# Victarry/Image-Generation-models

Measured on AMD Instinct MI355X. Metric: ddpm_cifar10_32x32_train_images_per_sec, higher is better.
Workload: dtype bf16; 1 GPU; DDPM CIFAR-10 32x32, UNet 128/1-2-4, T=1000 (BASELINE configs[1]): train step B=128/GPU + hipGraph denoise step B=64; per_gpu_batch=128, global_batch=128, parallelism=dp1, step_launch=hipGraph replay, denoise_batch=64, rccl_ranks=1, state_finite=True, matmul=bf16 MFMA, fp32 accumulate

## Files before the change

### image-generation-models_amd/csrc/conv_pw.hip

```cpp
#include "tr_common.h"

#ifndef MI_PW_PABL
#define MI_PW_PABL 0
#endif
#ifndef MI_PW_GNSABL
#define MI_PW_GNSABL 0
#endif
#ifndef MI_PW_FXABL
#define MI_PW_FXABL 0
#endif
#ifdef MI_PW_TIMING
__device__ uint32_t g_pw_ts[1024 * 4 * 5 * 64];
__device__ __forceinline__ uint32_t pw_wlane(uint32_t val, uint32_t lane, uint32_t v) {
    uint32_t keep;
    asm volatile("s_mov_b32 %1, m0\n\ts_mov_b32 m0, %3\n\ts_nop 0\n\tv_writelane_b32 %0, %2, m0\n\ts_mov_b32 m0, %1"
                 : "+v"(v), "=&s"(keep) : "s"(__builtin_amdgcn_readfirstlane(val)), "s"(__builtin_amdgcn_readfirstlane(lane)));
    return v;
}
extern "C" int mi_debug_pw_ts(uint32_t* host_out) { return (int)hipMemcpyFromSymbol(host_out, HIP_SYMBOL(g_pw_ts), sizeof(g_pw_ts)); }
#endif

namespace {

typedef uint32_t u32x2 __attribute__((ext_vector_type(2)));
// ... 1436 lines not shown
    auto unit = [&](int jt, auto chc, auto setc) {
        constexpr int ch = decltype(chc)::value, set = decltype(setc)::value;
        const bool last_unit = ch == NCH - 1 && jt + 1 >= jt1;
        if (!last_unit) {
            if constexpr (ch + 1 < NCH) load_wu(jt, ch + 1, std::integral_constant<int, set ^ 1>{});
            else load_wu(jt + 1, 0, std::integral_constant<int, set ^ 1>{});
        }
        bf16x8 XC[2][NBLK];
#pragma unroll
        for (int i = 0; i < NBLK; ++i) XC[0][i] = lds_b128p(xa[i] + ch * XB);
        static_for<0, 8>([&](auto uc) {
            constexpr int u = decltype(uc)::value;
            if constexpr (u + 1 < 8) {
                constexpr int un = u + 1;
#pragma unroll
                for (int i = 0; i < NBLK; ++i) XC[un & 1][i] = lds_b128p((xa[i] ^ ((un & 3) * 32)) + (un >> 2) * XH + ch * XB);
            }
#pragma unroll
            for (int i = 0; i < NBLK; ++i)
                acc[i] = __builtin_amdgcn_mfma_f32_32x32x16_bf16(__builtin_bit_cast(bf16x8, WB[set][u]), XC[u & 1][i], acc[i], 0, 0, 0);
            __builtin_amdgcn_sched_barrier(0);
        });
        if constexpr (ch == NCH - 1) {
            const int n0 = jt * 128;
            if (n0 + 32 * wv < a.Nc) {
#pragma unroll
                for (int rq = 0; rq < 4; ++rq) {
                    const int ck = 8 * wv + 2 * rq + (l >> 5);
                    f32x4 bq = {0.f, 0.f, 0.f, 0.f};
                    if (a.bias) bq = *reinterpret_cast<const f32x4*>(a.bias + n0 + 4 * ck);
#pragma unroll
                    for (int i = 0; i < NBLK; ++i) {
                        const int p = i * 32 + (l & 31);
                        *(lds_u32x2n*)(uintptr_t)(lds0 + STG + p * 256 + ((ck ^ ((p & 15) << 1)) << 3)) =
                            u32x2{pack_bf16(acc[i][4 * rq] + bq.x, acc[i][4 * rq + 1] + bq.y), pack_bf16(acc[i][4 * rq + 2] + bq.z, acc[i][4 * rq + 3] + bq.w)};
                    }
                }
            }
#pragma unroll
            for (int i = 0; i < NBLK; ++i)
#pragma unroll
                for (int r = 0; r < 16; ++r) acc[i][r] = 0.f;
        }
        asm volatile("s_waitcnt vmcnt(0)" ::: "memory");
        static_for<0, 8>([&](auto uc) { landed16(WB[set ^ 1][decltype(uc)::value]); });
        if constexpr (ch == NCH - 1) {
            const int n0 = jt * 128;
            __syncthreads();
            {
                const int j = t & 15, col = n0 + 8 * j;
                if (col < a.Nc) {
#pragma unroll
                    for (int it = 0; it < PXT / 16; ++it) {
                        const int p = it * 16 + (t >> 4);
                        const u32x4 o = *(lds_u32x4n*)(uintptr_t)(lds0 + STG + p * 256 + (((2 * j) ^ ((p & 15) << 1)) << 3));
                        *reinterpret_cast<u32x4*>(a.y + ((size_t)m0 + p) * a.ldy + col) = o;
                    }
                }
            }
            __syncthreads();
        }
    };
    auto cotile = [&](int jt, auto jpc) {
        constexpr int JP = decltype(jpc)::value;
        static_for<0, NCH>([&](auto chc) {
            constexpr int ch = decltype(chc)::value;
            unit(jt, chc, std::integral_constant<int, (JP * NCH + ch) & 1>{});
        });
    };
    for (int jt = jt0; jt < jt1; jt += 2) {
        cotile(jt, std::integral_constant<int, 0>{});
        if (jt + 1 < jt1) cotile(jt + 1, std::integral_constant<int, 1>{});
    }
}

struct GtClass { unsigned long long dyq, dxq, wtq; int ntap, ao, bo, pad_; };
struct GtArgs {
    const uint16_t* x; const uint16_t* w; const float* bias; const float* res; void* y; uint16_t* y16; int ldy16;
    int M, K, Nc, ldx, ldy, ldr, accumulate, gx, gy;
    int IH, IW, lgGW, lgGHW, si, so, OH, OW;
    GtClass cls[4];
};

template <bool OUT16, int PXT, bool F32 = false>
__global__ __launch_bounds__(256, 2) void conv_gt_kernel(const GtArgs a) {
    MI_PRIO_UP();
    static_assert(!F32 || !OUT16, "exact-fp32 mode writes fp32");
    constexpr int ESZ = F32 ? 4 : 2, EPP = 16 / ESZ, HCH = 8 * EPP;
    extern __shared__ __attribute__((aligned(16))) uint8_t lds_raw[];
    const uint32_t lds0 = (uint32_t)(uintptr_t)lds_raw;
    constexpr int NBLK = PXT / 32;
    constexpr int XH = PXT * 128;
    constexpr int XB = 2 * XH;
    const int t = threadIdx.x, l = t & 63;
    const int wv = __builtin_amdgcn_readfirstlane(t >> 6);
    int bx = blockIdx.x, by = blockIdx.y;
    if (a.gy > 1 && a.gx % 8 == 0) {
        const int id = blockIdx.x, xcd = id & 7, slot = id >> 3;
        bx = xcd * (a.gx >> 3) + slot / a.gy; by = slot % a.gy;
    }
    const GtClass cl = a.cls[blockIdx.z];
    const int m0 = bx * PXT, n0 = by * 128;
    const int NB = a.Nc >> 5, KQ = a.K / (2 * EPP), kc64 = a.K / HCH;
    const int nhc = cl.ntap * kc64, nchunks = (nhc + 1) >> 1;
    const bool live = n0 + 32 * wv < a.Nc;
    const int nb = min((n0 >> 5) + wv, NB - 1);

    int pbase[NBLK], iy0[NBLK], ix0[NBLK];
#pragma unroll
    for (int j = 0; j < NBLK; ++j) {
        const int m = m0 + 8 * (wv + 4 * j) + (l >> 3);
        const int n = m >> a.lgGHW, r = m & ((1 << a.lgGHW) - 1);
        pbase[j] = n * a.IH * a.IW; iy0[j] = (r >> a.lgGW) * a.si; ix0[j] = (r & ((1 << a.lgGW) - 1)) * a.si;
    }
    const uint8_t* zero = reinterpret_cast<const uint8_t*>(g_zero_page3) + (l & 7) * 16;
    auto stage_x = [&](int ch) {
#pragma unroll
        for (int h = 0; h < 2; ++h) {
            const int hc = min(2 * ch + h, 2 * nchunks - 1);
            const bool pad_half = hc >= nhc;
            const int hcc = min(hc, nhc - 1), tp = hcc / kc64, c0 = (hcc - tp * kc64) * HCH;
            const int dy = (int)((cl.dyq >> (4 * tp)) & 15) - 8, dx = (int)((cl.dxq >> (4 * tp)) & 15) - 8;
#pragma unroll
            for (int j = 0; j < NBLK; ++j) {
                const int px = 8 * (wv + 4 * j) + (l >> 3);
                const int iy = iy0[j] + dy, ix = ix0[j] + dx;
                const bool ok = !pad_half && (unsigned)iy < (unsigned)a.IH && (unsigned)ix < (unsigned)a.IW;
                size_t off = (size_t)(pbase[j] + iy * a.IW + ix) * a.ldx + c0 + ((l & 7) ^ ((px >> 1) & 7)) * EPP;
                asm volatile("" : "+v"(off));
                const uint8_t* src = ok ? reinterpret_cast<const uint8_t*>(a.x) + off * ESZ : zero;
                glds16(src, lds0 + (ch & 1) * XB + h * XH + (wv + 4 * j) * 1024);
            }
        }
    };
    const uint8_t* wbase = reinterpret_cast<const uint8_t*>(a.w) + (size_t)nb * KQ * 1024;
    const uint32_t tap_bytes = (uint32_t)NB * KQ * 1024;
    const uint32_t wl16 = l * 16;
    u32x4 WB[2][8];
    auto load_w = [&](int ch, auto setc) {
        constexpr int set = decltype(setc)::value;
        static_for<0, 2>([&](auto hcst) {
            constexpr int h = decltype(hcst)::value;
            const int hcc = min(2 * min(ch, nchunks - 1) + h, nhc - 1), tp = hcc / kc64, c0 = (hcc - tp * kc64) * HCH;
            const int wt = (int)((cl.wtq >> (4 * tp)) & 15);
            const uint64_t q = (uint64_t)(uintptr_t)(wbase + (size_t)wt * tap_bytes + (size_t)(c0 / (2 * EPP)) * 1024);
            const uint32_t lo = __builtin_amdgcn_readfirstlane((uint32_t)q), hi = __builtin_amdgcn_readfirstlane((uint32_t)(q >> 32));
            const uint64_t sb = ((uint64_t)hi << 32) | lo;
            static_for<0, 4>([&](auto uc) { gload16s<decltype(uc)::value * 1024>(WB[set][4 * h + decltype(uc)::value], sb, wl16); });
        });
    };
    uint32_t xa[NBLK];
#pragma unroll
    for (int i = 0; i < NBLK; ++i) {
        const int px = i * 32 + (l & 31);
        xa[i] = lds0 + px * 128 + (((l >> 5) * 16) ^ (((px >> 1) & 7) * 16));
    }
    f32x16 acc[NBLK];
#pragma unroll
    for (int i = 0; i < NBLK; ++i)
#pragma unroll
        for (int r = 0; r < 16; ++r) acc[i][r] = 0.f;

    stage_x(0);
    load_w(0, std::integral_constant<int, 0>{});
    asm volatile("s_waitcnt vmcnt(0)" ::: "memory");
    static_for<0, 8>([&](auto uc) { landed16(WB[0][decltype(uc)::value]); });
    auto chunk = [&](int ch, auto setc) {
        constexpr int set = decltype(setc)::value;
        asm volatile("s_waitcnt lgkmcnt(0)" ::: "memory");
        __builtin_amdgcn_s_barrier();
        asm volatile("" ::: "memory");
        if (ch + 1 < nchunks) {
            stage_x(ch + 1);
            load_w(ch + 1, std::integral_constant<int, set ^ 1>{});
        }
        const uint32_t xb = (ch & 1) * XB;
        bf16x8 XC[2][NBLK];
#pragma unroll
        for (int i = 0; i < NBLK; ++i) XC[0][i] = lds_b128p(xa[i] + xb);
        static_for<0, 8>([&](auto uc) {
            constexpr int u = decltype(uc)::value;
            if constexpr (u + 1 < 8) {
                constexpr int un = u + 1;
#pragma unroll
                for (int i = 0; i < NBLK; ++i) XC[un & 1][i] = lds_b128p((xa[i] ^ ((un & 3) * 32)) + (un >> 2) * XH + xb);
            }
#pragma unroll
            for (int i = 0; i < NBLK; ++i) {
                if constexpr (F32) {
                    const f32x4 wv4 = __builtin_bit_cast(f32x4, WB[set][u]), xv4 = __builtin_bit_cast(f32x4, XC[u & 1][i]);
#pragma unroll
                    for (int jj = 0; jj < 4; ++jj) acc[i] = __builtin_amdgcn_mfma_f32_32x32x2f32(wv4[jj], xv4[jj], acc[i], 0, 0, 0);
                } else
                acc[i] = __builtin_amdgcn_mfma_f32_32x32x16_bf16(__builtin_bit_cast(bf16x8, WB[set][u]), XC[u & 1][i], acc[i], 0, 0, 0);
            }
            __builtin_amdgcn_sched_barrier(0);
        });
        asm volatile("s_waitcnt vmcnt(0)" ::: "memory");
        static_for<0, 8>([&](auto uc) { landed16(WB[set ^ 1][decltype(uc)::value]); });
    };
    for (int ch = 0; ch < nchunks; ch += 2) {
        chunk(ch, std::integral_constant<int, 0>{});
        if (ch + 1 < nchunks) chunk(ch + 1, std::integral_constant<int, 1>{});
    }

    __syncthreads();
    typedef __attribute__((address_space(3))) f32x4 lds_f32x4;
    if (live) {
#pragma unroll
        for (int i = 0; i < NBLK; ++i) {
            const int p = i * 32 + (l & 31);
#pragma unroll
            for (int rq = 0; rq < 4; ++rq) {
                const int ck = 8 * wv + 2 * rq + (l >> 5);
                *(lds_f32x4*)(uintptr_t)(lds0 + p * 512 + ((ck ^ (p & 31)) << 4)) =
                    f32x4{acc[i][4 * rq], acc[i][4 * rq + 1], acc[i][4 * rq + 2], acc[i][4 * rq + 3]};
            }
        }
    }
    __syncthreads();
    const int j = t & 15, col = n0 + 8 * j;
    if (col >= a.Nc) return;
    f32x4 b0 = {0.f, 0.f, 0.f, 0.f}, b1 = b0;
    if (a.bias) { b0 = *reinterpret_cast<const f32x4*>(a.bias + col); b1 = *reinterpret_cast<const f32x4*>(a.bias + col + 4); }
#pragma unroll
    for (int it = 0; it < PXT / 16; ++it) {
        const int p = it * 16 + (t >> 4);
        const int mm = m0 + p, n = mm >> a.lgGHW, r = mm & ((1 << a.lgGHW) - 1);
        const size_t m = ((size_t)n * a.OH + (r >> a.lgGW) * a.so + cl.ao) * a.OW + (r & ((1 << a.lgGW) - 1)) * a.so + cl.bo;
        f32x4 v0 = *(lds_f32x4*)(uintptr_t)(lds0 + p * 512 + (((2 * j) ^ (p & 31)) << 4)) + b0;
        f32x4 v1 = *(lds_f32x4*)(uintptr_t)(lds0 + p * 512 + (((2 * j + 1) ^ (p & 31)) << 4)) + b1;
        if (a.res) {
            v0 += *reinterpret_cast<const f32x4*>(a.res + m * a.ldr + col);
            v1 += *reinterpret_cast<const f32x4*>(a.res + m * a.ldr + col + 4);
        }
        if constexpr (OUT16) {
            uint16_t* yp = reinterpret_cast<uint16_t*>(a.y) + m * a.ldy + col;
            if (a.accumulate) {
                const u32x4 o = *reinterpret_cast<const u32x4*>(yp);
                v0 += f32x4{__uint_as_float(o.x << 16), __uint_as_float(o.x & 0xffff0000u), __uint_as_float(o.y << 16), __uint_as_float(o.y & 0xffff0000u)};
                v1 += f32x4{__uint_as_float(o.z << 16), __uint_as_float(o.z & 0xffff0000u), __uint_as_float(o.w << 16), __uint_as_float(o.w & 0xffff0000u)};
            }
            *reinterpret_cast<u32x4*>(yp) = u32x4{pack_bf16(v0.x, v0.y), pack_bf16(v0.z, v0.w), pack_bf16(v1.x, v1.y), pack_bf16(v1.z, v1.w)};
        } else {
            float* yp = reinterpret_cast<float*>(a.y) + m * a.ldy + col;
            if (a.accumulate) { v0 += *reinterpret_cast<const f32x4*>(yp); v1 += *reinterpret_cast<const f32x4*>(yp + 4); }
            *reinterpret_cast<f32x4*>(yp) = v0;
            *reinterpret_cast<f32x4*>(yp + 4) = v1;
            if (a.y16)
                *reinterpret_cast<u32x4*>(a.y16 + m * a.ldy16 + col) =
                    u32x4{pack_bf16(v0.x, v0.y), pack_bf16(v0.z, v0.w), pack_bf16(v1.x, v1.y), pack_bf16(v1.z, v1.w)};
        }
    }
}

bool pw1_ok(const MiConvDesc* d, bool f32 = false, bool in32 = false) {
    if (in32) {
        if (d->KH != 1 || d->KW != 1 || d->pad != 0 || d->stride != 1 || d->mode != 1 || d->IH != d->OH || d->IW != d->OW) return false;
        if (d->K % 128 || d->K1 % 128 || d->K1 <= 0 || d->K1 > d->K || d->Nc % 64 || d->ldx % 4 || (d->K1 != d->K && d->ldx2 % 4)) return false;
        return ((long)d->N * d->OH * d->OW) % 128 == 0;
    }
    if (f32) {
        if (d->KH != 1 || d->KW != 1 || d->pad != 0 || d->stride != 1 || d->mode != 0 || d->IH != d->OH || d->IW != d->OW) return false;
        if (d->K % 64 || d->K1 % 64 || d->K1 <= 0 || d->K1 > d->K || d->Nc % 64 || d->ldx % 4 || (d->K1 != d->K && d->ldx2 % 4)) return false;
        return ((long)d->N * d->OH * d->OW) % 128 == 0;
    }
    if (d->KH != 1 || d->KW != 1 || d->pad != 0 || d->stride != 1 || d->mode != 1) return false;
    if (d->IH != d->OH || d->IW != d->OW) return false;
    if (d->K % 128 || d->K1 % 128 || d->K1 <= 0 || d->K1 > d->K || d->Nc % 64 || d->ldx % 8 || (d->K1 != d->K && d->ldx2 % 8)) return false;
    return ((long)d->N * d->OH * d->OW) % 128 == 0;
}

struct PwGn { const float* sums; const float* gamma; const float* beta; const float* temb; int ldt, G; float eps; };

static int pw_launch(const char* who, const MiConvDesc* d, const void* x, const void* x2, const void* w_frag_bf16, const float* bias,
                     const float* residual, void* y, int out_bf16, int var, float* gsum, const float* coef, void* stream,
                     const PwGn* gn = nullptr, bool in32 = false, bool f32 = false) {
    PwArgs a{};
    if (!d || !x || !w_frag_bf16 || !y) return mi_set_error(-1, "%s: null argument", who);
    const int pt = pw_pick_tile(d, var, &a.TH, &a.TI, in32, f32, &a.ksplit);
    if (!pt) return mi_set_error(-1, "%s: descriptor not supported by the private-weight-stream conv kernel", who);
    int dev_ = 0;
    (void)hipGetDevice(&dev_);
    if (a.ksplit > 1) {
        uint8_t* ws = reinterpret_cast<uint8_t*>(g_pw_sk_ws[dev_ & 63].load(std::memory_order_acquire));
        a.sk_flag = reinterpret_cast<int*>(ws); a.sk_part = reinterpret_cast<float*>(ws + PW_SK_FLAG_BYTES);
#ifdef MI_PW_SK_ABL
        a.sk_flag = nullptr;
#endif
    }
    if (d->K1 != d->K && !x2) return mi_set_error(-1, "%s: two-source split without x2", who);
    if ((((uintptr_t)x | (uintptr_t)(x2 ? x2 : x) | (uintptr_t)w_frag_bf16) & 15) != 0) return mi_set_error(-1, "%s: operands must be 16-byte aligned", who);
    if (d->ldy % 8 || (residual && d->ldr % 4)) return mi_set_error(-1, "%s: output pixel stride must be a multiple of 8, the residual's of 4", who);
    if (var >= 2 && (a.TI != 1 || d->K1 != d->K))
        return mi_set_error(-1, "%s: the fused variants need one image per tile and one source", who);
    if (var == 2 && (!coef || ((uintptr_t)coef & 15)))
        return mi_set_error(-1, "%s: the fused variant needs a 16-byte aligned coefficient tensor", who);
    if (var == 3) {
        if (!gn || !gn->sums || !gn->gamma || !gn->beta || gn->G <= 0 || d->K % gn->G || (d->K / gn->G) % 16 || d->K / gn->G > 64 || d->K / gn->G == 48)
            return mi_set_error(-1, "%s: sums, gamma, beta; K / G in {16, 32, 64}", who);
        if ((((uintptr_t)gn->gamma | (uintptr_t)gn->beta | (uintptr_t)gn->sums) & 7) || ((uintptr_t)gn->sums & 15) || (gn->temb && (((uintptr_t)gn->temb & 15) || gn->ldt % 4)))
            return mi_set_error(-1, "%s: misaligned GroupNorm operands", who);
        a.sums = gn->sums; a.gamma = gn->gamma; a.beta = gn->beta; a.temb = gn->temb; a.ldt = gn->ldt; a.cpg = d->K / gn->G;
        a.cpg_magic = pw_magic(a.cpg); a.ng = gn->G; a.hw = d->OH * d->OW; a.eps = gn->eps; a.icnt = 1.0 / (MI_GSUM_SCALE * (double)a.hw * (double)a.cpg);
    }
    if (var == 1 && (!gsum || d->Nc % 16)) return mi_set_error(-1, "%s: GroupNorm sums need Nc %% 16 == 0 and a sum buffer", who);
    a.x = (const uint16_t*)x; a.x2 = (const uint16_t*)(x2 ? x2 : x); a.w = (const uint16_t*)w_frag_bf16; a.bias = bias; a.res = residual; a.y = y;
    a.N = d->N; a.H = d->OH; a.W = d->OW; a.K = d->K; a.Nc = d->Nc; a.K1 = d->K1; a.ldx = d->ldx; a.ldx2 = x2 ? d->ldx2 : d->ldx;
    a.ldy = d->ldy; a.ldr = d->ldr; a.accumulate = d->accumulate; a.flip = d->transposed ? 1 : 0;
    a.gsum = gsum; a.coef = coef;
// ... 369 lines not shown
    a.ln_out = (uint16_t*)ln_bf16; a.ldl = ldl;
    hipStream_t st = (hipStream_t)stream;
#define MI_LNPW1_GO(PX, NC, G) do { \
        static MiPerDevice once_; \
        once_.run([] { (void)hipFuncSetAttribute((const void*)ln_conv1x1_pw_kernel<PX, NC, G>, hipFuncAttributeMaxDynamicSharedMemorySize, (int)lnpw1_lds(PX, NC)); }); \
        a.gx = a.M / PX; \
        hipLaunchKernelGGL((ln_conv1x1_pw_kernel<PX, NC, G>), dim3((unsigned)(a.gx * (G ? a.gy : 1))), dim3(256), lnpw1_lds(PX, NC), st, a); } while (0)
#define MI_LNPW1_PICK(PX, NC) do { if (a.M / PX < 512) MI_LNPW1_GO(PX, NC, true); else MI_LNPW1_GO(PX, NC, false); } while (0)
    if (d->K == 128) { if (a.M / 128 >= 512) MI_LNPW1_GO(128, 1, false); else MI_LNPW1_PICK(64, 1); }
    else if (d->K == 256) MI_LNPW1_PICK(64, 2);
    else MI_LNPW1_PICK(64, 4);
#undef MI_LNPW1_PICK
#undef MI_LNPW1_GO
    MI_LAUNCH_CHECK();
    return 0;
}

static int ilog2_exact(int v) { int lg = 0; while ((1 << lg) < v) ++lg; return (1 << lg) == v ? lg : -1; }

static bool gt_plan(const MiConvDesc* d, GtArgs& a, int* ncls, int* pxt) {
    if (!d || (d->mode != 1 && d->mode != 0) || d->K1 != d->K || d->K % 64 || d->Nc % 64 || d->ldx % (d->mode == 1 ? 8 : 4)) return false;
    const int k = d->KH, s = d->stride, p = d->pad;
    if (d->KW != k || k * k > 16 || k < 1 || (s != 1 && s != 2) || p < 0 || p > 7) return false;
    if ((long)d->Nc * d->K * (d->mode == 1 ? 2 : 4) * k * k >= (1L << 31)) return false;
    int GH, GW;
    *ncls = 0;
    if (!d->transposed) {
        if (d->OH != (d->IH + 2 * p - k) / s + 1 || d->OW != (d->IW + 2 * p - k) / s + 1) return false;
        GH = d->OH; GW = d->OW; a.si = s; a.so = 1;
        GtClass c{};
        for (int ky = 0; ky < k; ++ky)
            for (int kx = 0; kx < k; ++kx) {
                const int tp = c.ntap++;
                c.dyq |= (unsigned long long)(ky - p + 8) << (4 * tp); c.dxq |= (unsigned long long)(kx - p + 8) << (4 * tp);
                c.wtq |= (unsigned long long)(ky * k + kx) << (4 * tp);
            }
        a.cls[(*ncls)++] = c;
    } else {
        if (d->OH != s * d->IH || d->OW != s * d->IW) return false;
        GH = d->OH / s; GW = d->OW / s; a.si = 1; a.so = s;
        for (int cy = 0; cy < s; ++cy)
            for (int cx = 0; cx < s; ++cx) {
                GtClass c{};
                c.ao = cy; c.bo = cx;
                for (int ky = (cy + p) % s; ky < k; ky += s)
                    for (int kx = (cx + p) % s; kx < k; kx += s) {
                        const int dy = (cy + p - ky) / s, dx = (cx + p - kx) / s;
                        if (dy < -8 || dy > 7 || dx < -8 || dx > 7) return false;
                        const int tp = c.ntap++;
                        c.dyq |= (unsigned long long)(dy + 8) << (4 * tp); c.dxq |= (unsigned long long)(dx + 8) << (4 * tp);
                        c.wtq |= (unsigned long long)(ky * k + kx) << (4 * tp);
                    }
                if (c.ntap == 0) return false;
                a.cls[(*ncls)++] = c;
            }
    }
    a.lgGW = ilog2_exact(GW); a.lgGHW = ilog2_exact(GH * GW);
    if (a.lgGW < 0 || a.lgGHW < 0) return false;
    a.M = d->N * GH * GW; a.K = d->K; a.Nc = d->Nc; a.IH = d->IH; a.IW = d->IW; a.OH = d->OH; a.OW = d->OW;
    if (a.M % 64) return false;
    a.gy = (d->Nc + 127) / 128;
    const bool small = a.M % 128 != 0 || (long)(a.M / 128) * a.gy * *ncls < 256;
    *pxt = small ? 64 : 128;
    a.gx = a.M / *pxt;
    return true;
}
extern "C" int mi_conv_gt_supported(const MiConvDesc* d) {
    GtArgs a{};
    int ncls, pxt;
    return gt_plan(d, a, &ncls, &pxt) ? 1 : 0;
}
static int gt_launch(const MiConvDesc* d, const void* x, const void* w_frag, const float* bias, const float* residual,
                     void* y, int out_bf16, void* y_bf16, int ldy16, void* stream);
extern "C" int mi_conv_gt(const MiConvDesc* d, const void* x, const void* w_frag, const float* bias, const float* residual,
                          void* y, int out_bf16, void* stream) {
    return gt_launch(d, x, w_frag, bias, residual, y, out_bf16, nullptr, 0, stream);
}
extern "C" int mi_conv_gt_dual(const MiConvDesc* d, const void* x, const void* w_frag, const float* bias, const float* residual,
                               float* y, void* y_bf16, int ldy16, void* stream) {
    MI_REQUIRE(y_bf16 && ldy16 % 8 == 0 && (((uintptr_t)y_bf16) & 15) == 0 && d && !d->accumulate && d->mode == 1,
               "bf16 copy: bf16 mode, 16-byte aligned, ldy16 % 8 == 0, no accumulate");
    return gt_launch(d, x, w_frag, bias, residual, y, 0, y_bf16, ldy16, stream);
}
static int gt_launch(const MiConvDesc* d, const void* x, const void* w_frag, const float* bias, const float* residual,
                     void* y, int out_bf16, void* y_bf16, int ldy16, void* stream) {
    MI_REQUIRE(d && x && w_frag && y, "null argument");
    GtArgs a{};
    int ncls, pxt;
    MI_REQUIRE(gt_plan(d, a, &ncls, &pxt), "descriptor not supported by the tap-gather kernel (one source, K and Nc % 64 == 0, "
               "k * k <= 16 taps, stride 1 / 2, power-of-two grids, N*GH*GW % 64 == 0)");
    MI_REQUIRE((((uintptr_t)x | (uintptr_t)w_frag) & 15) == 0, "operands must be 16-byte aligned");
    MI_REQUIRE(d->ldy % 8 == 0 && (!residual || d->ldr % 4 == 0), "pixel strides: y % 8, residual % 4");
    MI_REQUIRE(d->mode == 1 || !out_bf16, "the exact-fp32 kernel writes fp32");
    a.x = (const uint16_t*)x; a.w = (const uint16_t*)w_frag; a.bias = bias; a.res = residual; a.y = y; a.y16 = (uint16_t*)y_bf16; a.ldy16 = ldy16;
    a.ldx = d->ldx; a.ldy = d->ldy; a.ldr = d->ldr; a.accumulate = d->accumulate;
    dim3 grid((unsigned)a.gx, (unsigned)a.gy, (unsigned)ncls);
    if (a.gy > 1 && a.gx % 8 == 0) grid = dim3((unsigned)(a.gx * a.gy), 1, (unsigned)ncls);
    hipStream_t st = (hipStream_t)stream;
#define MI_GT_GO(O16, PX, F) do { \
        static MiPerDevice once_; \
        once_.run([] { (void)hipFuncSetAttribute((const void*)conv_gt_kernel<O16, PX, F>, hipFuncAttributeMaxDynamicSharedMemorySize, 64 * 1024); }); \
        hipLaunchKernelGGL((conv_gt_kernel<O16, PX, F>), grid, dim3(256), (size_t)(PX == 128 ? 64 : 32) * 1024, st, a); } while (0)
    if (d->mode == 0) { if (pxt == 128) MI_GT_GO(false, 128, true); else MI_GT_GO(false, 64, true); }
    else if (pxt == 128) { if (out_bf16) MI_GT_GO(true, 128, false); else MI_GT_GO(false, 128, false); }
    else { if (out_bf16) MI_GT_GO(true, 64, false); else MI_GT_GO(false, 64, false); }
#undef MI_GT_GO
    MI_LAUNCH_CHECK();
    return 0;
}
extern "C" int mi_conv_gt_tile(const MiConvDesc* d, int* pxt, int* ncls) {
    GtArgs a{};
    return gt_plan(d, a, ncls, pxt) ? 0 : -1;
}
```

### image-generation-models_amd/src/ops/lib.py

```python
from __future__ import annotations

import ctypes as C
import os

_PKG_ROOT = os.path.dirname(os.path.dirname(os.path.dirname(os.path.abspath(__file__))))
_LIB = None


def library_path() -> str:
    return os.environ.get("MI_DDPM_LIB", os.path.join(_PKG_ROOT, "lib", "libmi_ddpm.so"))


class MiConvDesc(C.Structure):
    _fields_ = [(n, C.c_int) for n in (
        "N", "IH", "IW", "OH", "OW", "K", "Nc", "KH", "KW", "stride", "pad", "transposed", "w_kn", "mode",
        "K1", "ldx", "ldx2", "ldy", "ldr", "accumulate")]


class MiWgradDesc(C.Structure):
    _fields_ = [(n, C.c_int) for n in (
        "N", "GH", "GW", "DH", "DW", "Ci", "Cj", "KH", "KW", "stride", "pad", "gather_i", "mode", "I1",
        "ldp", "ldp2", "ldq")]


class MiGnDesc(C.Structure):
    _fields_ = [("N", C.c_int), ("HW", C.c_int), ("C", C.c_int), ("G", C.c_int), ("eps", C.c_float),
                ("ldx", C.c_int), ("ldy", C.c_int), ("ldr", C.c_int)]


class MiRowSum(C.Structure):
    _fields_ = [("src", C.c_void_p), ("dst", C.c_void_p), ("rows", C.c_int), ("cols", C.c_int), ("ld", C.c_int), ("pad_", C.c_int)]


WGRAD_STORE = 1


class MiPcnnConvDesc(C.Structure):
    _fields_ = ([(n, C.c_int) for n in ("N", "H", "W", "Cin", "ldx", "Cout", "ldy", "ntaps")]
                + [(n, C.c_int * 25) for n in ("tap_dy", "tap_dx", "tap_w")]
                + [(n, C.c_int) for n in ("w_sk", "w_sc", "C2", "ldx2", "w2_sk", "w2_sc", "epi", "elu_in", "accumulate", "gate_C",
                                          "ldpre", "ldcond", "ldr", "ldaux", "mode")])


ROWSUM_MAX = 16
LATENT_DISC_NMAX = 1024
LATENT_DISC_LN_NMAX = 65536
_P, _I, _F, _Z = C.c_void_p, C.c_int, C.c_float, C.c_size_t

SIGNATURES = {
    "mi_conv_igemm": [C.POINTER(MiConvDesc), _P, _P, _P, _P, _P, _P, _P],
    "mi_conv_igemm_bf16w": [C.POINTER(MiConvDesc), _P, _P, _P, _P, _P, _P, _P],
    "mi_conv_igemm_bf16w_io": [C.POINTER(MiConvDesc), _P, _P, _P, _P, _P, _P, _I, _P],
    "mi_conv_igemm_bf16w_io_supported": [C.POINTER(MiConvDesc)],
    "mi_conv_gt_supported": [C.POINTER(MiConvDesc)],
    "mi_conv_gt_tile": [C.POINTER(MiConvDesc), C.POINTER(C.c_int), C.POINTER(C.c_int)],
    "mi_conv_gt": [C.POINTER(MiConvDesc), _P, _P, _P, _P, _P, _I, _P],
    "mi_conv_gt_dual": [C.POINTER(MiConvDesc), _P, _P, _P, _P, _P, _P, _I, _P],
    "mi_conv_igemm_tile": [C.POINTER(MiConvDesc), C.POINTER(C.c_int), C.POINTER(C.c_int)],
    "mi_conv3x3_bf16w": [C.POINTER(MiConvDesc), _P, _P, _P, _P, _P, _P, _P],
    "mi_conv3x3_bf16w_supported": [C.POINTER(MiConvDesc)],
    "mi_conv3x3_bf16w_uses_splitk": [C.POINTER(MiConvDesc)],
    "mi_conv3x3_bf16w_tile": [C.POINTER(MiConvDesc), _I, C.POINTER(C.c_int), C.POINTER(C.c_int), C.POINTER(C.c_int)],
    "mi_conv3x3_wgrad_tile": [C.POINTER(MiWgradDesc), C.POINTER(C.c_int), C.POINTER(C.c_int)],
    "mi_debug_wgrad3x3_phase": [_I],
    "mi_conv3x3_wgrad_tr_supported": [C.POINTER(MiWgradDesc)],
    "mi_conv3x3_wgrad_tr_splits": [C.POINTER(MiWgradDesc)],
    "mi_conv3x3_wgrad_tr": [C.POINTER(MiWgradDesc), _P, _P, _P, _P, _P, _Z, _P],
    "mi_conv3x3_wgrad_tr_batch": [_I, C.POINTER(MiWgradDesc), C.POINTER(_P), C.POINTER(_P), C.POINTER(_P), C.POINTER(_P), _P, _Z, _P],
    "mi_debug_wgrad_tr_phase": [_I],
    "mi_conv1x1_wgrad_tr_supported": [C.POINTER(MiWgradDesc), _I],
    "mi_conv1x1_wgrad_tr_batch": [_I, C.POINTER(MiWgradDesc), C.POINTER(_I), C.POINTER(_P), C.POINTER(_P), C.POINTER(_P), C.POINTER(_P),
                                  C.POINTER(_P), _P, _Z, _P],
    "mi_debug_wgrad1x1_tr_phase": [_I],
    "mi_conv_s2_wgrad_tr_supported": [C.POINTER(MiWgradDesc)],
    "mi_conv_s2_wgrad_tr_batch": [_I, C.POINTER(MiWgradDesc), C.POINTER(_P), C.POINTER(_P), C.POINTER(_P), _P, _Z, _P],
    "mi_conv_s2_wgrad_f32_supported": [C.POINTER(MiWgradDesc)],
    "mi_conv_s2_wgrad_f32": [C.POINTER(MiWgradDesc), _P, _P, _P, _P, _Z, _P],
    "mi_debug_wgrad_s2_tr_phase": [_I],
    "mi_conv3x3_wgrad_tr_batch_ex": [_I, C.POINTER(MiWgradDesc), C.POINTER(_P), C.POINTER(_P), C.POINTER(_P), C.POINTER(_P), _P, _Z, _P, C.c_uint],
    "mi_conv1x1_wgrad_tr_batch_ex": [_I, C.POINTER(MiWgradDesc), C.POINTER(_I), C.POINTER(_P), C.POINTER(_P), C.POINTER(_P), C.POINTER(_P),
                                     C.POINTER(_P), _P, _Z, _P, C.c_uint],
    "mi_conv_s2_wgrad_tr_batch_ex": [_I, C.POINTER(MiWgradDesc), C.POINTER(_P), C.POINTER(_P), C.POINTER(_P), _P, _Z, _P, C.c_uint],
    "mi_zero_ranges": [_P, _I, _P, _P],
    "mi_debug_spin": [_I, _I, _P, _Z, _I, _P],
    "mi_debug_clock_probe": [_I, _I, _P, _P],
    "mi_pack_weights_tile": [],
    "mi_conv3x3_bf16w_io_gnsums": [C.POINTER(MiConvDesc), _P, _P, _P, _P, _P, _P, _I, _P, _P],
    "mi_gn_coef_from_sums": [_I, _I, _I, _I, _F, _P, _P, _P, _P, _I, _P, _P, _P],
    "mi_gn_mish_apply_sums": [C.POINTER(MiGnDesc), _P, _P, _P, _P, _P, _I, _P, _P, _I, _P, _I, _P, _P],
    "mi_conv3x3_bf16w_io_dual": [C.POINTER(MiConvDesc), _P, _P, _P, _P, _P, _P, _P, _I, _I, _P],
    "mi_conv3x3_gn_mish_sums": [C.POINTER(MiConvDesc), _P, _P, _P, _P, _P, _I, _I, _F, _P, _P, _P, _I, _P],
    "mi_debug_wgrad1x1_tr_blocks": [_I],
    "mi_debug_wgrad_tr_blocks": [_I],
    "mi_conv3x3_bf16w_io": [C.POINTER(MiConvDesc), _P, _P, _P, _P, _P, _P, _I, _P],
    "mi_conv3x3_wgrad_io": [C.POINTER(MiWgradDesc), _P, _P, _P, _P, _P, _P, _Z, _I, _P],
    "mi_gn_mish_fwd_io": [C.POINTER(MiGnDesc), _P, _P, _P, _P, _I, _P, _P, _P, _I, _P],
    "mi_gn_mish_fwd_dual": [C.POINTER(MiGnDesc), _P, _P, _P, _P, _I, _P, _P, _P, _I, _P, _I, _P],
    "mi_f32_to_bf16": [_Z, _I, _P, _I, _P, _I, _P],
    "mi_f32_to_bf16_colsum": [_Z, _I, _P, _I, _P, _I, _P, _P, _Z, _P],
    "mi_gn_mish_bwd_io": [C.POINTER(MiGnDesc), _P, _P, _P, _P, _P, _I, _P, _I, _P, _P, _P, _I, _P, _I, _P],
    "mi_pack_weights_bf16": [_I, _P, _I, _P, _P, _P, _P, _P, _P],
    "mi_conv3x3_pw_supported": [C.POINTER(MiConvDesc)],
    "mi_conv3x3_pw_tile": [C.POINTER(MiConvDesc)],
    "mi_debug_conv_pw_tile": [_I],
    "mi_debug_conv_pw_auto256": [_I],
    "mi_debug_conv1x1_pw_nloop": [_I],
    "mi_conv3x3_pw_f32_tile": [C.POINTER(MiConvDesc)],
    "mi_conv3x3_pw_f32": [C.POINTER(MiConvDesc), _P, _P, _P, _P, _P, _P, _P],
    "mi_conv1x1_pw_x32_supported": [C.POINTER(MiConvDesc)],
    "mi_conv1x1_pw_x32": [C.POINTER(MiConvDesc), _P, _P, _P, _P, _P, _P, _I, _P],
    "mi_conv_pw_set_splitk_workspace": [_P, C.c_size_t],
    "mi_conv3x3_pw_splitk": [C.POINTER(MiConvDesc), _I, _I],
    "mi_debug_conv_pw_splitk": [_I],
    "mi_ln_conv1x1_pw_supported": [C.POINTER(MiConvDesc)],
    "mi_ln_conv1x1_pw": [C.POINTER(MiConvDesc), _P, _P, _P, C.c_float, _P, _P, _P, _P],
    "mi_ln_conv1x1_pw_dual": [C.POINTER(MiConvDesc), _P, _P, _P, C.c_float, _P, _P, _P, _P, _I, _P],
    "mi_conv1x1_pw_f32_supported": [C.POINTER(MiConvDesc)],
    "mi_conv1x1_pw_f32": [C.POINTER(MiConvDesc), _P, _P, _P, _P, _P, _P, _P],
    "mi_pack_weights_f32frag": [_I, _P, _I, _P, _P, _P, _P],
    "mi_conv3x3_pw_x32_supported": [C.POINTER(MiConvDesc)],
    "mi_conv3x3_pw_x32_tile": [C.POINTER(MiConvDesc)],
    "mi_conv3x3_pw_x32": [C.POINTER(MiConvDesc), _P, _P, _P, _P, _P, _P, _I, _P, _P],
    "mi_conv3x3_pw": [C.POINTER(MiConvDesc), _P, _P, _P, _P, _P, _P, _I, _P],
    "mi_conv3x3_pw_gn_mish_supported": [C.POINTER(MiConvDesc)],
    "mi_conv1x1_pw_supported": [C.POINTER(MiConvDesc)],
    "mi_conv1x1_pw": [C.POINTER(MiConvDesc), _P, _P, _P, _P, _P, _P, _I, _P, _I, _P],
    "mi_conv3x3_pw_gnsums": [C.POINTER(MiConvDesc), _P, _P, _P, _P, _P, _P, _I, _P, _P],
    "mi_conv3x3_pw_gn_mish": [C.POINTER(MiConvDesc), _P, _P, _P, _P, _P, _I, _P],
    "mi_conv3x3_pw_gn_mish_sums": [C.POINTER(MiConvDesc), _P, _P, _P, _P, _P, _I, _I, _F, _P, _P, _P, _I, _P],
    "mi_conv3x3_pw_x32_gn_mish_supported": [C.POINTER(MiConvDesc)],
    "mi_conv3x3_pw_x32_gn_mish_tile": [C.POINTER(MiConvDesc)],
    "mi_conv3x3_pw_gn_mish_tile": [C.POINTER(MiConvDesc)],
    "mi_conv3x3_pw_x32_gn_mish": [C.POINTER(MiConvDesc), _P, _P, _P, _P, _P, _I, _P],
    "mi_conv3x3_pw_x32_gn_mish_sums": [C.POINTER(MiConvDesc), _P, _P, _P, _P, _P, _I, _I, _F, _P, _P, _P, _I, _P],
    "mi_gn_stats_coef": [C.POINTER(MiGnDesc), _P, _P, _P, _P, _I, _P, _P, _I, _P],
    "mi_conv3x3_gn_mish_supported": [C.POINTER(MiConvDesc)],
    "mi_conv3x3_gn_mish_tile": [C.POINTER(MiConvDesc), C.POINTER(C.c_int), C.POINTER(C.c_int)],
    "mi_conv3x3_gn_mish": [C.POINTER(MiConvDesc), _P, _P, _P, _P, _P, _I, _P],
# ... 176 lines not shown
```

### include/mi_ddpm.h

```cpp
#ifndef MI_DDPM_H
#define MI_DDPM_H
#include <stddef.h>
#include <stdint.h>

#ifdef __cplusplus
extern "C" {
#endif

#define MI_ABI_VERSION 4
#define MI_MODE_FP32 0
#define MI_MODE_BF16 1

int mi_abi_version(void);
const char* mi_last_error(void);

typedef struct MiConvDesc {
    int N;
    int IH, IW;
    int OH, OW;
    int K;
    int Nc;
    int KH, KW, stride, pad;
    int transposed;
    int w_kn;
    int mode;
    int K1;
    int ldx, ldx2, ldy, ldr;
    int accumulate;
} MiConvDesc;

int mi_conv_igemm(const MiConvDesc* d, const float* x, const float* x2, const float* w,
                  const float* bias, const float* residual, float* y, void* stream);

int mi_conv_igemm_bf16w(const MiConvDesc* d, const float* x, const float* x2, const void* w_nk_bf16,
                        const float* bias, const float* residual, float* y, void* stream);
int mi_conv_igemm_bf16w_io_supported(const MiConvDesc* d);
int mi_conv_igemm_bf16w_io(const MiConvDesc* d, const void* x, const void* x2, const void* w_nk_bf16,
                           const float* bias, const float* residual, float* y, int x_is_bf16, void* stream);
int mi_conv_igemm_tile(const MiConvDesc* d, int* bm, int* bn);

int mi_conv_gt_supported(const MiConvDesc* d);
int mi_conv_gt_tile(const MiConvDesc* d, int* pixels_per_workgroup, int* classes);
int mi_conv_gt(const MiConvDesc* d, const void* x, const void* w_frag, const float* bias, const float* residual,
               void* y, int out_bf16, void* stream);
int mi_conv_gt_dual(const MiConvDesc* d, const void* x, const void* w_frag, const float* bias, const float* residual,
                    float* y, void* y_bf16, int ldy16, void* stream);

int mi_conv3x3_bf16w(const MiConvDesc* d, const float* x, const float* x2, const void* w_nk_bf16,
                     const float* bias, const float* residual, float* y, void* stream);
int mi_conv3x3_bf16w_supported(const MiConvDesc* d);
int mi_conv3x3_bf16w_uses_splitk(const MiConvDesc* d);
int mi_conv3x3_bf16w_tile(const MiConvDesc* d, int io, int* bm, int* ck, int* sk);
int mi_conv3x3_bf16w_io(const MiConvDesc* d, const void* x, const void* x2, const void* w_nk_bf16,
                        const float* bias, const float* residual, void* y, int io, void* stream);
int mi_conv3x3_bf16w_io_dual(const MiConvDesc* d, const void* x, const void* x2, const void* w_nk_bf16, const float* bias,
                             const float* residual, float* y, void* y_bf16, int ldy16, int io, void* stream);
int mi_conv3x3_bf16w_io_gnsums(const MiConvDesc* d, const void* x, const void* x2, const void* w_nk_bf16, const float* bias,
                               const float* residual, void* y, int io, float* gsum, void* stream);
int mi_gn_coef_from_sums(int N, int C, int G, int HW, float eps, const float* sums, const float* gamma, const float* beta,
                         const float* temb, int ldt, float* stats, float* coef, void* stream);
int mi_conv3x3_gn_mish_sums(const MiConvDesc* d, const void* x, const float* sums, const float* gamma, const float* beta,
                            const float* temb, int ldt, int G, float eps, const void* w_nk_bf16, const float* bias, void* y,
                            int io, void* stream);
int mi_conv3x3_gn_mish_supported(const MiConvDesc* d);
int mi_conv3x3_gn_mish_tile(const MiConvDesc* d, int* bm, int* ck);
int mi_conv3x3_gn_mish(const MiConvDesc* d, const void* x, const float* coef, const void* w_nk_bf16, const float* bias,
                       void* y, int io, void* stream);
int mi_pack_weights_tile(void);
int mi_pack_weights_bf16(int nent, const void* entries_dev, int total_tiles, const float* master,
                         void* wd_bf16, void* wf_bf16, void* wdq_bf16, void* wfq_bf16, void* stream);
int mi_conv3x3_pw_supported(const MiConvDesc* d);
int mi_conv3x3_pw_x32_supported(const MiConvDesc* d);
int mi_conv3x3_pw_x32_tile(const MiConvDesc* d);
int mi_conv3x3_pw_x32(const MiConvDesc* d, const float* x, const float* x2, const void* w_frag_bf16, const float* bias,
                      const float* residual, void* y, int out_bf16, float* gsum, void* stream);
int mi_conv3x3_pw_f32_tile(const MiConvDesc* d);
int mi_conv3x3_pw_f32(const MiConvDesc* d, const float* x, const float* x2, const float* w_frag_f32, const float* bias,
                      const float* residual, float* y, void* stream);
int mi_conv1x1_pw_x32_supported(const MiConvDesc* d);
int mi_conv1x1_pw_x32(const MiConvDesc* d, const float* x, const float* x2, const void* w_frag_bf16, const float* bias,
                      const float* residual, void* y, int out_bf16, void* stream);
int mi_conv_pw_set_splitk_workspace(void* ws, size_t bytes);
int mi_conv3x3_pw_splitk(const MiConvDesc* d, int var, int in32);
int mi_debug_conv_pw_splitk(int mode);
int mi_ln_conv1x1_pw_supported(const MiConvDesc* d);
int mi_ln_conv1x1_pw(const MiConvDesc* d, const float* x, const float* ln_g, const float* ln_b, float eps, const void* w_frag_bf16,
                     const float* bias, void* y_bf16, void* stream);
int mi_ln_conv1x1_pw_dual(const MiConvDesc* d, const float* x, const float* ln_g, const float* ln_b, float eps, const void* w_frag_bf16,
                          const float* bias, void* y_bf16, void* ln_bf16, int ldl, void* stream);
int mi_conv1x1_pw_f32_supported(const MiConvDesc* d);
int mi_conv1x1_pw_f32(const MiConvDesc* d, const float* x, const float* x2, const float* w_frag_f32, const float* bias,
                      const float* residual, float* y, void* stream);
int mi_pack_weights_f32frag(int nent, const void* entries_dev, int total_tiles, const float* master, float* wdq32, float* wfq32,
                            void* stream);
int mi_debug_conv_pw_tile(int pt);
int mi_debug_conv_pw_auto256(int min_workgroups);
int mi_debug_conv1x1_pw_nloop(int on);
int mi_conv3x3_pw_tile(const MiConvDesc* d);
int mi_conv3x3_pw(const MiConvDesc* d, const void* x, const void* x2, const void* w_frag_bf16, const float* bias,
                  const float* residual, void* y, int out_bf16, void* stream);
int mi_conv3x3_pw_gnsums(const MiConvDesc* d, const void* x, const void* x2, const void* w_frag_bf16, const float* bias,
                         const float* residual, void* y, int out_bf16, float* gsum, void* stream);
int mi_conv3x3_pw_gn_mish_supported(const MiConvDesc* d);
int mi_conv3x3_pw_gn_mish_tile(const MiConvDesc* d);
int mi_conv3x3_pw_gn_mish(const MiConvDesc* d, const void* x, const float* coef, const void* w_frag_bf16, const float* bias,
                          void* y, int out_bf16, void* stream);
int mi_conv3x3_pw_gn_mish_sums(const MiConvDesc* d, const void* x, const float* sums, const float* gamma, const float* beta,
                               const float* temb, int ldt, int G, float eps, const void* w_frag_bf16, const float* bias,
                               void* y, int out_bf16, void* stream);
int mi_conv3x3_pw_x32_gn_mish_supported(const MiConvDesc* d);
int mi_conv3x3_pw_x32_gn_mish_tile(const MiConvDesc* d);
int mi_conv3x3_pw_x32_gn_mish(const MiConvDesc* d, const float* x, const float* coef, const void* w_frag_bf16, const float* bias,
                              void* y, int out_bf16, void* stream);
int mi_conv3x3_pw_x32_gn_mish_sums(const MiConvDesc* d, const float* x, const float* sums, const float* gamma, const float* beta,
                                   const float* temb, int ldt, int G, float eps, const void* w_frag_bf16, const float* bias,
                                   void* y, int out_bf16, void* stream);
int mi_conv1x1_pw_supported(const MiConvDesc* d);
int mi_conv1x1_pw(const MiConvDesc* d, const void* x, const void* x2, const void* w_frag_bf16, const float* bias, const float* residual,
                  void* y, int out_bf16, void* y_bf16, int ldy16, void* stream);

int mi_conv_small_cin_fwd(int ks, int N, int H, int W, int Cin, int Cout, const float* x, int ldx, const float* w,
                          const float* bias, float* y, int ldy, void* stream);
int mi_conv_small_cin_wgrad(int ks, int N, int H, int W, int Cin, int Cout, const float* x, int ldx, const float* dy,
                            int lddy, float* dW, void* workspace, size_t ws_bytes, void* stream);
size_t mi_conv_small_wgrad_workspace(int outputs);
// ... 342 lines not shown
```

Before: 27360 images/s.

## Split K-loop of conv_gt kernel across wave teams with LDS reduction

Adds an intra-workgroup split-K: the conv_gt kernel can launch 2 or 4 teams of four waves, each team processing an interleaved subset of K chunks into its own LDS double buffer, then reducing partial accumulators through LDS before the epilogue. A heuristic enables teams in bf16 mode when the grid is small (at most 256 workgroups) and the chunk count is large, targeting underutilized CUs on small-batch launches. It costs more LDS per workgroup, a reduction pass, and possibly lower occupancy.

```diff
diff --git a/image-generation-models_amd/csrc/conv_pw.hip b/image-generation-models_amd/csrc/conv_pw.hip
--- a/image-generation-models_amd/csrc/conv_pw.hip
+++ b/image-generation-models_amd/csrc/conv_pw.hip
@@ -1542,10 +1542,11 @@
     GtClass cls[4];
 };
 
-template <bool OUT16, int PXT, bool F32 = false>
-__global__ __launch_bounds__(256, 2) void conv_gt_kernel(const GtArgs a) {
+template <bool OUT16, int PXT, bool F32 = false, int TEAMS = 1>
+__global__ __launch_bounds__(256 * TEAMS, (TEAMS > 2 ? TEAMS : 2)) void conv_gt_kernel(const GtArgs a) {
     MI_PRIO_UP();
     static_assert(!F32 || !OUT16, "exact-fp32 mode writes fp32");
+    static_assert((TEAMS == 1 || TEAMS == 2 || TEAMS == 4) && TEAMS * PXT * 512 <= 128 * 1024 && PXT % (16 * TEAMS) == 0, "teams: 1, 2 or 4 within 128 KB of LDS");
     constexpr int ESZ = F32 ? 4 : 2, EPP = 16 / ESZ, HCH = 8 * EPP;
     extern __shared__ __attribute__((aligned(16))) uint8_t lds_raw[];
     const uint32_t lds0 = (uint32_t)(uintptr_t)lds_raw;
@@ -1553,7 +1554,8 @@
     constexpr int XH = PXT * 128;
     constexpr int XB = 2 * XH;
     const int t = threadIdx.x, l = t & 63;
-    const int wv = __builtin_amdgcn_readfirstlane(t >> 6);
+    const int wvg = __builtin_amdgcn_readfirstlane(t >> 6);
+    const int wv = TEAMS == 1 ? wvg : wvg & 3, team = TEAMS == 1 ? 0 : wvg >> 2;
     int bx = blockIdx.x, by = blockIdx.y;
     if (a.gy > 1 && a.gx % 8 == 0) {
         const int id = blockIdx.x, xcd = id & 7, slot = id >> 3;
@@ -1563,6 +1565,8 @@
     const int m0 = bx * PXT, n0 = by * 128;
     const int NB = a.Nc >> 5, KQ = a.K / (2 * EPP), kc64 = a.K / HCH;
     const int nhc = cl.ntap * kc64, nchunks = (nhc + 1) >> 1;
+    const int niter = (nchunks + TEAMS - 1) / TEAMS;
+    const uint32_t ldst = lds0 + team * (2 * XB);
     const bool live = n0 + 32 * wv < a.Nc;
     const int nb = min((n0 >> 5) + wv, NB - 1);
 
@@ -1574,10 +1578,11 @@
         pbase[j] = n * a.IH * a.IW; iy0[j] = (r >> a.lgGW) * a.si; ix0[j] = (r & ((1 << a.lgGW) - 1)) * a.si;
     }
     const uint8_t* zero = reinterpret_cast<const uint8_t*>(g_zero_page3) + (l & 7) * 16;
-    auto stage_x = [&](int ch) {
+    auto stage_x = [&](int it) {
+        const int ch = team + it * TEAMS;
 #pragma unroll
         for (int h = 0; h < 2; ++h) {
-            const int hc = min(2 * ch + h, 2 * nchunks - 1);
+            const int hc = 2 * ch + h;
             const bool pad_half = hc >= nhc;
             const int hcc = min(hc, nhc - 1), tp = hcc / kc64, c0 = (hcc - tp * kc64) * HCH;
             const int dy = (int)((cl.dyq >> (4 * tp)) & 15) - 8, dx = (int)((cl.dxq >> (4 * tp)) & 15) - 8;
@@ -1589,7 +1594,7 @@
                 size_t off = (size_t)(pbase[j] + iy * a.IW + ix) * a.ldx + c0 + ((l & 7) ^ ((px >> 1) & 7)) * EPP;
                 asm volatile("" : "+v"(off));
                 const uint8_t* src = ok ? reinterpret_cast<const uint8_t*>(a.x) + off * ESZ : zero;
-                glds16(src, lds0 + (ch & 1) * XB + h * XH + (wv + 4 * j) * 1024);
+                glds16(src, ldst + (it & 1) * XB + h * XH + (wv + 4 * j) * 1024);
             }
         }
     };
@@ -1597,8 +1602,9 @@
     const uint32_t tap_bytes = (uint32_t)NB * KQ * 1024;
     const uint32_t wl16 = l * 16;
     u32x4 WB[2][8];
-    auto load_w = [&](int ch, auto setc) {
+    auto load_w = [&](int it, auto setc) {
         constexpr int set = decltype(setc)::value;
+        const int ch = team + it * TEAMS;
         static_for<0, 2>([&](auto hcst) {
             constexpr int h = decltype(hcst)::value;
             const int hcc = min(2 * min(ch, nchunks - 1) + h, nhc - 1), tp = hcc / kc64, c0 = (hcc - tp * kc64) * HCH;
@@ -1613,7 +1619,7 @@
 #pragma unroll
     for (int i = 0; i < NBLK; ++i) {
         const int px = i * 32 + (l & 31);
-        xa[i] = lds0 + px * 128 + (((l >> 5) * 16) ^ (((px >> 1) & 7) * 16));
+        xa[i] = ldst + px * 128 + (((l >> 5) * 16) ^ (((px >> 1) & 7) * 16));
     }
     f32x16 acc[NBLK];
 #pragma unroll
@@ -1630,7 +1636,7 @@
         asm volatile("s_waitcnt lgkmcnt(0)" ::: "memory");
         __builtin_amdgcn_s_barrier();
         asm volatile("" ::: "memory");
-        if (ch + 1 < nchunks) {
+        if (ch + 1 < niter) {
             stage_x(ch + 1);
             load_w(ch + 1, std::integral_constant<int, set ^ 1>{});
         }
@@ -1659,33 +1665,53 @@
         asm volatile("s_waitcnt vmcnt(0)" ::: "memory");
         static_for<0, 8>([&](auto uc) { landed16(WB[set ^ 1][decltype(uc)::value]); });
     };
-    for (int ch = 0; ch < nchunks; ch += 2) {
+    for (int ch = 0; ch < niter; ch += 2) {
         chunk(ch, std::integral_constant<int, 0>{});
-        if (ch + 1 < nchunks) chunk(ch + 1, std::integral_constant<int, 1>{});
+        if (ch + 1 < niter) chunk(ch + 1, std::integral_constant<int, 1>{});
     }
 
     __syncthreads();
     typedef __attribute__((address_space(3))) f32x4 lds_f32x4;
-    if (live) {
+    constexpr int ET = PXT * 512;
+    auto put_acc = [&](uint32_t base) {
 #pragma unroll
         for (int i = 0; i < NBLK; ++i) {
             const int p = i * 32 + (l & 31);
 #pragma unroll
             for (int rq = 0; rq < 4; ++rq) {
                 const int ck = 8 * wv + 2 * rq + (l >> 5);
-                *(lds_f32x4*)(uintptr_t)(lds0 + p * 512 + ((ck ^ (p & 31)) << 4)) =
+                *(lds_f32x4*)(uintptr_t)(base + p * 512 + ((ck ^ (p & 31)) << 4)) =
                     f32x4{acc[i][4 * rq], acc[i][4 * rq + 1], acc[i][4 * rq + 2], acc[i][4 * rq + 3]};
             }
         }
-    }
+    };
+    if constexpr (TEAMS > 1) {
+        if (live && team > 0) put_acc(lds0 + team * ET);
+        __syncthreads();
+        if (live && team == 0) {
+#pragma unroll
+            for (int k = 1; k < TEAMS; ++k)
+#pragma unroll
+                for (int i = 0; i < NBLK; ++i) {
+                    const int p = i * 32 + (l & 31);
+#pragma unroll
+                    for (int rq = 0; rq < 4; ++rq) {
+                        const int ck = 8 * wv + 2 * rq + (l >> 5);
+                        const f32x4 v = *(lds_f32x4*)(uintptr_t)(lds0 + k * ET + p * 512 + ((ck ^ (p & 31)) << 4));
+                        acc[i][4 * rq] += v.x; acc[i][4 * rq + 1] += v.y; acc[i][4 * rq + 2] += v.z; acc[i][4 * rq + 3] += v.w;
+                    }
+                }
+        }
+    }
+    if (live && team == 0) put_acc(lds0);
     __syncthreads();
     const int j = t & 15, col = n0 + 8 * j;
     if (col >= a.Nc) return;
     f32x4 b0 = {0.f, 0.f, 0.f, 0.f}, b1 = b0;
     if (a.bias) { b0 = *reinterpret_cast<const f32x4*>(a.bias + col); b1 = *reinterpret_cast<const f32x4*>(a.bias + col + 4); }
 #pragma unroll
-    for (int it = 0; it < PXT / 16; ++it) {
-        const int p = it * 16 + (t >> 4);
+    for (int it = 0; it < PXT / (16 * TEAMS); ++it) {
+        const int p = it * 16 * TEAMS + (t >> 4);
         const int mm = m0 + p, n = mm >> a.lgGHW, r = mm & ((1 << a.lgGHW) - 1);
         const size_t m = ((size_t)n * a.OH + (r >> a.lgGW) * a.so + cl.ao) * a.OW + (r & ((1 << a.lgGW) - 1)) * a.so + cl.bo;
         f32x4 v0 = *(lds_f32x4*)(uintptr_t)(lds0 + p * 512 + (((2 * j) ^ (p & 31)) << 4)) + b0;
@@ -2221,6 +2247,28 @@
                "bf16 copy: bf16 mode, 16-byte aligned, ldy16 % 8 == 0, no accumulate");
     return gt_launch(d, x, w_frag, bias, residual, y, 0, y_bf16, ldy16, stream);
 }
+static int g_gt_force_teams = 0;
+static bool gt_teams_exist(const MiConvDesc* d, int pxt, int teams) {
+    return teams == 1 || (d->mode == 1 && (teams == 2 || (teams == 4 && pxt == 64)));
+}
+static int gt_teams(const MiConvDesc* d, const GtArgs& a, int ncls, int pxt) {
+    if (g_gt_force_teams) return gt_teams_exist(d, pxt, g_gt_force_teams) ? g_gt_force_teams : 0;
+    if (d->mode != 1 || (long)a.gx * a.gy * ncls > 256) return 1;
+    int most = 0;
+    for (int c = 0; c < ncls; ++c) { const int n = (a.cls[c].ntap * (a.K / 64) + 1) >> 1; most = n > most ? n : most; }
+    if (pxt == 64 && most >= 24) return 4;
+    return most >= 16 ? 2 : 1;
+}
+extern "C" int mi_debug_conv_gt_teams(int teams) {
+    if (teams != 0 && teams != 1 && teams != 2 && teams != 4) return mi_set_error(-1, "mi_debug_conv_gt_teams: 0, 1, 2 or 4");
+    g_gt_force_teams = teams;
+    return 0;
+}
+extern "C" int mi_conv_gt_teams(const MiConvDesc* d) {
+    GtArgs a{};
+    int ncls, pxt;
+    return gt_plan(d, a, &ncls, &pxt) ? gt_teams(d, a, ncls, pxt) : 0;
+}
 static int gt_launch(const MiConvDesc* d, const void* x, const void* w_frag, const float* bias, const float* residual,
                      void* y, int out_bf16, void* y_bf16, int ldy16, void* stream) {
     MI_REQUIRE(d && x && w_frag && y, "null argument");
@@ -2233,16 +2281,22 @@
     MI_REQUIRE(d->mode == 1 || !out_bf16, "the exact-fp32 kernel writes fp32");
     a.x = (const uint16_t*)x; a.w = (const uint16_t*)w_frag; a.bias = bias; a.res = residual; a.y = y; a.y16 = (uint16_t*)y_bf16; a.ldy16 = ldy16;
     a.ldx = d->ldx; a.ldy = d->ldy; a.ldr = d->ldr; a.accumulate = d->accumulate;
+    const int teams = gt_teams(d, a, ncls, pxt);
+    MI_REQUIRE(teams > 0, "mi_debug_conv_gt_teams: the forced team count has no instantiation for this launch (bf16 mode; 4 teams: 64-pixel tiles)");
     dim3 grid((unsigned)a.gx, (unsigned)a.gy, (unsigned)ncls);
     if (a.gy > 1 && a.gx % 8 == 0) grid = dim3((unsigned)(a.gx * a.gy), 1, (unsigned)ncls);
     hipStream_t st = (hipStream_t)stream;
-#define MI_GT_GO(O16, PX, F) do { \
+#define MI_GT_GO(O16, PX, F, T) do { \
         static MiPerDevice once_; \
-        once_.run([] { (void)hipFuncSetAttribute((const void*)conv_gt_kernel<O16, PX, F>, hipFuncAttributeMaxDynamicSharedMemorySize, 64 * 1024); }); \
-        hipLaunchKernelGGL((conv_gt_kernel<O16, PX, F>), grid, dim3(256), (size_t)(PX == 128 ? 64 : 32) * 1024, st, a); } while (0)
-    if (d->mode == 0) { if (pxt == 128) MI_GT_GO(false, 128, true); else MI_GT_GO(false, 64, true); }
-    else if (pxt == 128) { if (out_bf16) MI_GT_GO(true, 128, false); else MI_GT_GO(false, 128, false); }
-    else { if (out_bf16) MI_GT_GO(true, 64, false); else MI_GT_GO(false, 64, false); }
+        once_.run([] { (void)hipFuncSetAttribute((const void*)conv_gt_kernel<O16, PX, F, T>, hipFuncAttributeMaxDynamicSharedMemorySize, T * PX * 512); }); \
+        hipLaunchKernelGGL((conv_gt_kernel<O16, PX, F, T>), grid, dim3(256 * T), (size_t)(T * PX * 512), st, a); } while (0)
+#define MI_GT_OUT(PX, T) do { if (out_bf16) MI_GT_GO(true, PX, false, T); else MI_GT_GO(false, PX, false, T); } while (0)
+    if (d->mode == 0) { if (pxt == 128) MI_GT_GO(false, 128, true, 1); else MI_GT_GO(false, 64, true, 1); }
+    else if (pxt == 128) { if (teams == 2) MI_GT_OUT(128, 2); else MI_GT_OUT(128, 1); }
+    else if (teams == 4) MI_GT_OUT(64, 4);
+    else if (teams == 2) MI_GT_OUT(64, 2);
+    else MI_GT_OUT(64, 1);
+#undef MI_GT_OUT
 #undef MI_GT_GO
     MI_LAUNCH_CHECK();
     return 0;
diff --git a/image-generation-models_amd/src/ops/lib.py b/image-generation-models_amd/src/ops/lib.py
--- a/image-generation-models_amd/src/ops/lib.py
+++ b/image-generation-models_amd/src/ops/lib.py
@@ -54,6 +54,8 @@
     "mi_conv_igemm_bf16w_io_supported": [C.POINTER(MiConvDesc)],
     "mi_conv_gt_supported": [C.POINTER(MiConvDesc)],
     "mi_conv_gt_tile": [C.POINTER(MiConvDesc), C.POINTER(C.c_int), C.POINTER(C.c_int)],
+    "mi_conv_gt_teams": [C.POINTER(MiConvDesc)],
+    "mi_debug_conv_gt_teams": [_I],
     "mi_conv_gt": [C.POINTER(MiConvDesc), _P, _P, _P, _P, _P, _I, _P],
     "mi_conv_gt_dual": [C.POINTER(MiConvDesc), _P, _P, _P, _P, _P, _P, _I, _P],
     "mi_conv_igemm_tile": [C.POINTER(MiConvDesc), C.POINTER(C.c_int), C.POINTER(C.c_int)],
diff --git a/include/mi_ddpm.h b/include/mi_ddpm.h
--- a/include/mi_ddpm.h
+++ b/include/mi_ddpm.h
@@ -41,6 +41,8 @@
 
 int mi_conv_gt_supported(const MiConvDesc* d);
 int mi_conv_gt_tile(const MiConvDesc* d, int* pixels_per_workgroup, int* classes);
+int mi_conv_gt_teams(const MiConvDesc* d);
+int mi_debug_conv_gt_teams(int teams);
 int mi_conv_gt(const MiConvDesc* d, const void* x, const void* w_frag, const float* bias, const float* residual,
                void* y, int out_bf16, void* stream);
 int mi_conv_gt_dual(const MiConvDesc* d, const void* x, const void* w_frag, const float* bias, const float* residual,
```

Result: no change. 27470 images/s, median of 6 (+0.4%).
